# kocurvik/mdrp

Measured on AMD Instinct MI355X. Metric: image-pairs/sec (2000 corrs, 10k RANSAC iters), higher is better.
Workload: dtype f64

## Files before the change

### mdrp_amd/csrc/mdrp_capi.hip

```cpp
#include "../../include/mdrp.h"
#include "mdrp_kernels.h"
#include "mdrp_classic.h"
#ifdef MDRP_SPLIT_TU
#define MDRP_INST extern
#include "mdrp_instances.h"
namespace mdrp {
MDRP_INSTANCES_FINAL_64
MDRP_INSTANCES_FINAL_256
MDRP_INSTANCES_CLASSIC
}
#endif

#include <algorithm>
#include <cmath>
#include <cstdio>
#include <cstdlib>
#include <cstddef>
#include <cstring>
#include <functional>
#include <map>
#include <mutex>
#include <string>
#include <vector>

// ... 424 lines not shown
            int rc_;
            if ((rc_ = get_events(h, &v0, &v1, 5))) return rc_;
            HIPCHK(hipEventRecord(v0, st_));
            struct Stop { hipEvent_t e; hipStream_t s; ~Stop() { (void)hipEventRecord(e, s); } } stop_{v1, st_};
            PairState *st_p = h->st.as<PairState>() + p0;
            double *pts_p = h->pts.as<double>() + (size_t)p0 * n_max * PT_STRIDE;
            Model *models_p = h->models.as<Model>() + so;
            int32_t *inl_p = h->slot_inl.as<int32_t>() + so;
            if (classic) {
                const dim3 sgrid((r.chunk_len + 63) / 64, pc);
                if (kind == MDRP_SHARED_6PT)
                    hipLaunchKernelGGL(kc_solve<CLASSIC_SHARED>, sgrid, dim3(64), 0, st_, r, st_p, smp, pts_p, models_p, inl_p, tg, mc);
                else if (kind == MDRP_RELPOSE_5PT) {
                    const bool first_region = c == 0 && n_chunks > 1;
                    if (first_region && (size_t)sgrid.x > red5_first_blocks) { g_err = "5-point first chunk longer than its Reduce5 region"; return MDRP_ERR_INVALID; }
                    double *red5 = h->red5.as<double>() + ((first_region ? (size_t)batch * red5_blocks : 0) + (size_t)p0 * sgrid.x) * RED5_STRIDE * 64;
                    hipLaunchKernelGGL(kc_solve5_null, sgrid, dim3(64), SOLVE5N_LDS_BYTES, st_, r, st_p, smp, pts_p, red5);
                    hipLaunchKernelGGL(kc_solve5_reduce, sgrid, dim3(64), SOLVE5_LDS_BYTES, st_, r, st_p, red5);
                    hipLaunchKernelGGL(kc_solve5_roots, sgrid, dim3(64), SOLVE5B_LDS_BYTES, st_, r, st_p, smp, pts_p, red5, models_p, inl_p, tg, mc);
                }
                else
                    hipLaunchKernelGGL(kc_solve<CLASSIC_FUND>, sgrid, dim3(64), SOLVE7_LDS_BYTES, st_, r, st_p, smp, pts_p, models_p, inl_p, tg, mc);
                return MDRP_OK;
            }
            double *dep_p = h->dep.as<double>() + (size_t)p0 * n_max * 2;
#define MDRP_SOLVE_LAUNCH(S)                                                                                                   \
    hipLaunchKernelGGL(k_solve<S>, dim3((r.chunk_len + solve_threads(S) - 1) / solve_threads(S), pc), dim3(solve_threads(S)), 0, st_, r, st_p, smp, pts_p, dep_p, models_p, inl_p, tg, mc, 0, r.chunk_len)
            switch (r.solver) {
            case SOLVER_P3P: MDRP_SOLVE_LAUNCH(SOLVER_P3P); break;
            case SOLVER_SHIFT: MDRP_SOLVE_LAUNCH(SOLVER_SHIFT); break;
            case SOLVER_SHARED: MDRP_SOLVE_LAUNCH(SOLVER_SHARED); break;
            default: MDRP_SOLVE_LAUNCH(SOLVER_VARYING); break;
            }
#undef MDRP_SOLVE_LAUNCH
            return MDRP_OK;
        };
        auto sweep_chunk = [&](int c, int p0, int pc) -> int {
            RunParams r = rp;
            r.chunk_len = (int)lens[c]; r.chunk_off = offs[c]; r.batch = pc;
            const int len = r.chunk_len;
            const bool odd = c & 1;
            const size_t so = (size_t)p0 * rp.slot_stride;
            PairState *st_p = h->st.as<PairState>() + p0;
            const double *pts_p = h->pts.as<double>() + (size_t)p0 * n_max * PT_STRIDE;
            const Model *models_p = h->models.as<Model>() + so;
            uint32_t *tags_sc = (odd ? h->tags2_s : h->tags_s).as<uint32_t>() + so;
            int32_t *mcount_c = (odd ? h->model_count2 : h->model_count).as<int32_t>() + 2 * (size_t)p0;
            uint32_t *tags_c = (odd ? h->tags2 : h->tags).as<uint32_t>() + so;
            uint32_t *tags_v = h->tags_v.as<uint32_t>() + so;
            int32_t *surv1 = h->surv_count.as<int32_t>() + p0, *surv2 = h->surv2_count.as<int32_t>() + p0;
            hipEvent_t e0, e1;
            int rc_;
            if ((rc_ = get_events(h, &e0, &e1, 0))) return rc_;
            unsigned long long *cstats = reinterpret_cast<unsigned long long *>(cnt + 6);
            {
                hipEvent_t c0, c1;
                if ((rc_ = get_events(h, &c0, &c1, 1))) return rc_;
                const bool two_phase = !(it0 == 0 && c == 0);
                unsigned long long *cand_stat = h->cand_stat.as<unsigned long long>() + 2 * (size_t)p0;
                uint32_t *tags_u = tags_sc;
                int32_t *und_part = reinterpret_cast<int32_t *>((odd ? h->tags_s : h->tags2_s).as<uint32_t>() + so), *und_cnt = h->und_count.as<int32_t>() + 2 * (size_t)p0;
                const uint4 *rfrag_p = h->rfrag.as<uint4>() + (size_t)p0 * groups_max * 64;
                hipLaunchKernelGGL(k_count_plan, dim3(1), dim3(PLAN_THREADS), 0, s, pc, st_p, mcount_c, 2, CNT_WG_MODELS, h->cplan.as<int32_t>(),
                                   surv1, (const int32_t *)nullptr, two_phase ? und_cnt : (int32_t *)nullptr);
                const dim3 cgrid((unsigned)pc * (unsigned)((len * mps + CNT_WG_MODELS - 1) / CNT_WG_MODELS));
                HIPCHK(hipEventRecord(c0, s));
                MDRP_SWEEP_DISPATCH(k_count, kind, cgrid, dim3(CNT_THREADS), 0, s, r, st_p, rfrag_p, models_p,
                                    tags_c, mcount_c, h->cplan.as<int32_t>(), tags_v, surv1, cstats, (int32_t *)nullptr, (const int32_t *)nullptr,
                                    1, tags_u, und_part, und_cnt, (const int32_t *)nullptr, cand_stat);
                if (two_phase) {
                    hipLaunchKernelGGL(k_count_plan, dim3(1), dim3(PLAN_THREADS), 0, s, pc, st_p, und_cnt, 2, CNT_WG_MODELS, h->cplan.as<int32_t>(),
                                       (int32_t *)nullptr, (const int32_t *)nullptr, (int32_t *)nullptr);
                    MDRP_SWEEP_DISPATCH(k_count, kind, cgrid, dim3(CNT_THREADS), 0, s, r, st_p, rfrag_p, models_p,
                                        tags_u, und_cnt, h->cplan.as<int32_t>(), tags_v, surv1, cstats, (int32_t *)nullptr, (const int32_t *)nullptr,
                                        2, (uint32_t *)nullptr, (int32_t *)nullptr, (int32_t *)nullptr, und_part, cand_stat);
                    h->count_launches++;
                }
                HIPCHK(hipEventRecord(c1, s));
                h->count_launches++;
            }
            const uint32_t *surv_tags = tags_v;
            const int32_t *surv_cnt = surv1;
            if (use_bound && batch_call > 16 && !(it0 == 0 && c == 0)) {
                hipLaunchKernelGGL(k_count_plan, dim3(1), dim3(PLAN_THREADS), 0, s, pc, st_p, surv1, 1, BND_THREADS, h->cplan.as<int32_t>(), surv2, (const int32_t *)nullptr);
                const dim3 bgrid((unsigned)pc * (unsigned)((len * mps + BND_THREADS - 1) / BND_THREADS));
                unsigned long long *bstats = reinterpret_cast<unsigned long long *>(cnt + 12);
                hipEvent_t b0, b1;
                if ((rc_ = get_events(h, &b0, &b1, 4))) return rc_;
                HIPCHK(hipEventRecord(b0, s));
                MDRP_SWEEP_DISPATCH(k_bound, kind, bgrid, dim3(BND_THREADS), 0, s, r, st_p, pts_p, models_p, tags_v, surv1, h->cplan.as<int32_t>(), tags_c, surv2, bstats);
                HIPCHK(hipEventRecord(b1, s));
                surv_tags = tags_c; surv_cnt = surv2;
            }
            int32_t *plan = h->plan.as<int32_t>(), *totals = plan + 2 * (size_t)batch + 2;
            if (batch_call <= SCORE_WAVE_MAX_PAIRS) {
                hipLaunchKernelGGL(k_count_plan, dim3(1), dim3(PLAN_THREADS), 0, s, pc, st_p, surv_cnt, 1, SCW_THREADS / 64, plan, (int32_t *)nullptr, (const int32_t *)nullptr, (int32_t *)nullptr);
                hipLaunchKernelGGL(k_sort_tags, dim3(pc), dim3(256), 0, s, r, st_p, mcount_c, surv_cnt, surv_tags, tags_sc);
                HIPCHK(hipEventRecord(e0, s));
                const long long ub = (long long)pc * ((len * mps + SCW_THREADS / 64 - 1) / (SCW_THREADS / 64));
                const dim3 grid((unsigned)std::min<long long>(ub, (long long)h->num_cu * 32));
                MDRP_SWEEP_DISPATCH(k_score_w, kind, grid, dim3(SCW_THREADS), 0, s, r, st_p, pts_p, models_p, tags_sc, mcount_c,
                                    h->slot_score.as<double>() + so, h->slot_inl.as<int32_t>() + so, plan);
            } else {
                hipLaunchKernelGGL(k_sort_tags, dim3(pc), dim3(256), 0, s, r, st_p, mcount_c, surv_cnt, surv_tags, tags_sc);
                hipLaunchKernelGGL(k_plan, dim3(1), dim3(PLAN_THREADS), 0, s, pc, mcount_c, plan, totals);
                HIPCHK(hipEventRecord(e0, s));
                const dim3 grid((unsigned)pc * (unsigned)((len * mps + SCORE_THREADS - 1) / SCORE_THREADS));
                MDRP_SWEEP_DISPATCH(k_score, kind, grid, dim3(SCORE_THREADS), tile_bytes, s, r, st_p, pts_p, models_p, tags_sc, mcount_c,
                                    h->slot_score.as<double>() + so, h->slot_inl.as<int32_t>() + so, plan, totals);
            }
            HIPCHK(hipEventRecord(e1, s));
            h->sweep_launches++;
            Trigger *trig_p = h->triggers.as<Trigger>() + (size_t)p0 * trig_cap;
            unsigned long long *scan_stats = reinterpret_cast<unsigned long long *>(cnt + 10);
#define MDRP_SCAN(M, I) hipLaunchKernelGGL((k_scan<M, I>), dim3(pc), dim3(64), 0, s, r, st_p, h->slot_score.as<double>() + so, h->slot_inl.as<int32_t>() + so, trig_p, trig_cap, mcount_c, scan_stats)
            if (mps == 16) MDRP_SCAN(16, 1);
            else if (mps == 12) MDRP_SCAN(12, 1);
            else if (len >= 1024) MDRP_SCAN(4, 4);
            else MDRP_SCAN(4, 1);
#undef MDRP_SCAN
            return MDRP_OK;
        };
        bool solved1 = false;
        int swept0 = 0;
        if (host && it0 == 0) {
            const bool sliced = piped && n_chunks >= 2 && batch >= 2 * HOST_SLICE_PAIRS;
            const int sl = sliced ? HOST_SLICE_PAIRS : batch;
            for (int p0 = 0; p0 < batch; p0 += sl) {
                const int pc = std::min(sl, batch - p0);
                const size_t o2 = (size_t)2 * p0 * n_max, o1 = (size_t)p0 * n_max, n2 = sizeof(double) * 2 * (size_t)pc * n_max, n1 = sizeof(double) * (size_t)pc * n_max;
                hipStream_t cs = sliced ? h->copy_stream : s;
                HIPCHK(hipMemcpyAsync(const_cast<double *>(x1) + o2, host->x1 + o2, n2, hipMemcpyHostToDevice, cs));
                HIPCHK(hipMemcpyAsync(const_cast<double *>(x2) + o2, host->x2 + o2, n2, hipMemcpyHostToDevice, cs));
                if (host->d1 && host->d2) {
                    HIPCHK(hipMemcpyAsync(const_cast<double *>(d1) + o1, host->d1 + o1, n1, hipMemcpyHostToDevice, cs));
                    HIPCHK(hipMemcpyAsync(const_cast<double *>(d2) + o1, host->d2 + o1, n1, hipMemcpyHostToDevice, cs));
                }
                if (!sliced) { launch_prep(p0, pc, s); break; }
                HIPCHK(hipEventRecord(h->ev_copied, cs)); HIPCHK(hipStreamWaitEvent(aux, h->ev_copied, 0));
                if (p0 == 0) HIPCHK(hipStreamWaitEvent(aux, h->ev_tables, 0));
                launch_prep(p0, pc, aux);
                HIPCHK(hipEventRecord(h->ev_prepped, aux));
                if ((rc = issue_solve(1, aux, p0, pc))) return rc;
                const bool last = p0 + sl >= batch, last_but_one = !last && p0 + 2 * sl >= batch;
                if (last_but_one || last) HIPCHK(hipStreamWaitEvent(s, h->ev_prepped, 0));
                if (last_but_one) { swept0 = p0 + pc; if ((rc = issue_solve(0, s, 0, swept0)) || (rc = sweep_chunk(0, 0, swept0))) return rc; }
                if (last) { if ((rc = issue_solve(0, s, swept0, batch - swept0)) || (rc = sweep_chunk(0, swept0, batch - swept0))) return rc; swept0 = batch; }
            }
            if (sliced) { HIPCHK(hipEventRecord(h->ev_solved[1], aux)); solved1 = true; }
        }
        if (swept0 < batch && (rc = issue_solve(0, s, 0, batch))) return rc;
        if (piped) HIPCHK(hipEventRecord(h->ev_solved[0], s));
        for (int c = 0; c < n_chunks; ++c) {
            rp.chunk_len = (int)lens[c]; rp.chunk_off = offs[c];
            if (c == 0 && swept0 >= batch) {
                if (piped) HIPCHK(hipEventRecord(h->ev_scanned[0], s));
                continue;
            }
            if (piped && c + 1 < n_chunks && !(c == 0 && solved1)) {
                HIPCHK(hipStreamWaitEvent(aux, c == 0 ? h->ev_solved[0] : h->ev_scanned[c - 1], 0));
                if ((rc = issue_solve(c + 1, aux, 0, batch))) return rc;
                HIPCHK(hipEventRecord(h->ev_solved[c + 1], aux));
            }
            if (piped && c > 0) HIPCHK(hipStreamWaitEvent(s, h->ev_solved[c], 0));
            if (!piped && c > 0 && (rc = issue_solve(c, s, 0, batch))) return rc;
            if ((rc = sweep_chunk(c, 0, batch))) return rc;
            if (c + 1 < n_chunks) {
                if (piped) HIPCHK(hipEventRecord(h->ev_scanned[c], s));
                continue;
            }
            int32_t *lo_plan = h->work_pair.as<int32_t>();
            hipLaunchKernelGGL(k_lo_plan, dim3(1), dim3(PLAN_THREADS), 0, s, batch, h->st.as<PairState>(), (const int32_t *)nullptr, lo_plan);
            if (fuse_tail) {
// ... 683 lines not shown
```

### mdrp_amd/csrc/mdrp_kernels.h

```cpp
#pragma once
#include <hip/hip_runtime.h>
#include <float.h>
#include "mdrp_logtab.h"
#include "mdrp_math.h"

#ifdef MDRP_SECONDARY_TU
#define MDRP_GLOBAL static __global__
#else
#define MDRP_GLOBAL __global__
#endif

namespace mdrp {

constexpr int PT_STRIDE = 6;
#define MDRP_TILE_PTS 512
#define MDRP_SCORE_MINWAVES 4
constexpr int TILE_PTS = MDRP_TILE_PTS;
constexpr size_t SCORE_TILE_BYTES = (size_t)TILE_PTS * (PT_STRIDE * sizeof(double) + 4 * sizeof(float));
#define MDRP_P1F_UNROLL 8
#define MDRP_P1_UNROLL 4
constexpr int PRUNE_EVERY = 4;
#define MDRP_DENSE_KEY 40
#define MDRP_SOLVE_MINWAVES 2
#define MDRP_SCORE_THREADS 256
// ... 904 lines not shown
                if (g + 2 < A_TILE_GROUPS) {
#pragma unroll
                    for (int t = 0; t < CNT_TILES; t += 2) { test2(t); mfma2(f0, t); }
                } else {
#pragma unroll
                    for (int t = 0; t < CNT_TILES; t += 2) test2(t);
                }
            }
        }
        if (tile + 1 < t_hi) commit(buf ^ 1);
        __syncthreads();
    }
    if (idle) return;
    uint32_t *s_out = reinterpret_cast<uint32_t *>(&s_frag[wave][0][0]);
    const int swept = (t_hi - t_lo) * A_TILE_GROUPS * 16, real = min(max(n - t_lo * A_TILE_GROUPS * 16, 0), swept);
    const int pad = swept - real;
    const bool split_a = phase == 1 && t_hi < n_tiles;
    const int rest = split_a ? n - t_hi * A_TILE_GROUPS * 16 : 0;
#pragma unroll
    for (int t = 0; t < CNT_TILES; ++t) {
        float o = cand[t];
        o += __shfl_xor(o, 16, 64);
        o += __shfl_xor(o, 32, 64);
        if (ksl == 0) s_out[16 * t + col] = (uint32_t)((int)o - pad);
    }
    __builtin_amdgcn_fence(__ATOMIC_RELEASE, "wavefront");
    __builtin_amdgcn_wave_barrier();
    const long long rec_cnt = (long long)ps.best_min_cnt;
    const double rec_score = ps.best_min_score < DBL_MAX ? ps.best_min_score * (1.0 + 1e-12) : DBL_MAX;
#pragma unroll
    for (int r = 0; r < CNT_ROUNDS; ++r) {
        const int i = m0 + 64 * r + lane;
        const bool live = i < cnt;
        const int cnd_here = live ? (int)s_out[64 * r + lane] + part_r[r] : 0;
        const int cnd = cnd_here + rest;
        if (cand_stat && phase == 1 && !split_a && rec_cnt == 0 && !(ps.best_min_score < DBL_MAX)) {
            const int tot = wave_sum_i(cnd_here), lv = __popcll(__ballot(live));
            if (lane == 0 && lv) { atomicAdd(&cand_stat[2 * pair], (unsigned long long)tot); atomicAdd(&cand_stat[2 * pair + 1], (unsigned long long)lv * (unsigned long long)n); }
        }
        if (cand_out && live) cand_out[i] = cnd;
        const bool surv = live && ((long long)cnd > rec_cnt || thr * (double)(n - cnd) < rec_score);
        const unsigned long long ball = __ballot(surv);
        if (ball) {
            int base = 0;
            const int first = __ffsll((long long)ball) - 1;
            if (lane == first) base = atomicAdd(split_a ? &und_count[2 * pair] : &surv_count[pair], __popcll(ball));
            base = __shfl(base, first, 64);
            if (surv) {
                const size_t at = slot_base + base + __popcll(ball & ((1ull << lane) - 1ull));
                if (split_a) { tags_und[at] = slot_r[r]; und_part[at] = cnd_here; }
                else {
                    const uint32_t key = (uint32_t)min(PROBE_PTS, (int)(((long long)cnd * PROBE_PTS + n - 1) / n));
                    tags_surv[at] = slot_r[r] | (key << 24);
                }
            }
        }
    }
    if (stats && lane == 0 && wave == 0 && blk == 0) {
        if (phase != 2) atomicAdd(&stats[0], (unsigned long long)cnt * (unsigned long long)n);
        atomicAdd(&stats[1], (unsigned long long)(((cnt + 15) / 16) * 16) * (unsigned long long)swept);
    }
}

constexpr int BND_THREADS = 256;
#define MDRP_BND_TILE 256
constexpr int BND_TILE = MDRP_BND_TILE;

template <bool POSE, bool RAWF>
__device__ __forceinline__ void model_matrix(const Model &m, double E[9]) {
    if (RAWF) {
#pragma unroll
        for (int q = 0; q < 9; ++q) E[q] = reinterpret_cast<const double *>(&m)[q];
    } else {
        double R[9], Em[9];
        quat_to_R(m.q, R);
        essential_from_Rt(R, m.t, Em);
        if (POSE) {
#pragma unroll
            for (int q = 0; q < 9; ++q) E[q] = Em[q];
        } else fundamental_from_E(Em, m.f1, m.f2, E);
    }
}

template <bool POSE, bool RAWF = false>
__global__ __launch_bounds__(BND_THREADS, 4) void k_bound(RunParams rp, const PairState *__restrict__ st, const double *__restrict__ pts,
                                                          const Model *__restrict__ models, const uint32_t *__restrict__ tags_in,
                                                          const int32_t *__restrict__ cnt_in, const int32_t *__restrict__ plan,
                                                          uint32_t *__restrict__ tags_out,
                                                          int32_t *__restrict__ cnt_out, unsigned long long *__restrict__ stats,
                                                          double *__restrict__ dbg_lb = nullptr ,
                                                          int32_t *__restrict__ dbg_cnt_ub = nullptr) {
    __shared__ float4 s_rec[BND_TILE];
    struct Open { uint32_t tag; int32_t sane; float Ef[9], eC, eD, thr_dn, c0, c1; double lb; };
    __shared__ Open s_open[BND_THREADS];
    __shared__ int s_wave_open[BND_THREADS / 64];
    const int total = plan[rp.batch];
    const int w = blockIdx.x;
    if (w >= total) return;
    const int pair = plan_find(plan, rp.batch, w);
    const int blk = w - plan[pair];
    const PairState &ps = st[pair];
    const int n = ps.n, cnt = cnt_in[pair];
    const int tid = threadIdx.x, lane = tid & 63, wave = tid >> 6;
    const int i = blk * BND_THREADS + tid;
    bool open = i < cnt;
    const size_t slot_base = (size_t)pair * rp.slot_stride;
    const double thr = ps.sq_thr;
    uint32_t tag = 0;
    float Ef[9], eC = 0.f, eD = 1.f, thr_dn = 0.f;
    bool sane = false;
#pragma unroll
    for (int q = 0; q < 9; ++q) Ef[q] = 0.f;
    if (open) {
        tag = tags_in[slot_base + i];
        const Model m = models[slot_base + (tag & 0xFFFFFFu)];
        double E[9];
        model_matrix<POSE, RAWF>(m, E);
        sane = bound_setup32(E, ps.box, thr, Ef, eC, eD, thr_dn);
    }
    double total_lb = 0.0;
    f32x2 cnt2 = {0.f, 0.f};
    const float thr_cnt = (float)(thr * (1.0 + 1e-5)) * (1.0f + 1e-6f);
    const float BIG = 1.2089258e24f;
    const f32x2 nbig = {-BIG, -BIG}, kcnt = {thr_cnt * BIG, thr_cnt * BIG};
    const long long rec_cnt = (long long)ps.best_min_cnt;
    const double rec_score = ps.best_min_score < DBL_MAX ? ps.best_min_score * (1.0 + 1e-12) : DBL_MAX;
    float4 *s_pair = s_rec;
    const double *gp = pts + (size_t)pair * rp.n_max * PT_STRIDE;
    for (int t0 = 0; t0 < n; t0 += BND_TILE) {
        const int npts = min(BND_TILE, n - t0);
        __syncthreads();
        for (int j = tid; j < npts; j += BND_THREADS) {
            const double2 *src = reinterpret_cast<const double2 *>(gp + (size_t)(t0 + j) * PT_STRIDE);
            const double2 p0 = src[0], p1 = src[1];
            store_rec32(s_pair, j, p0.x, p0.y, p1.x, p1.y);
        }
        __syncthreads();
        if (__ballot(open)) {
            f32x2 Ev[9];
#pragma unroll
            for (int q = 0; q < 9; ++q) Ev[q] = (f32x2){Ef[q], Ef[q]};
            const f32x2 eDv = {eD, eD};
            const int npairs = npts >> 1;
            for (int j0 = 0; j0 < npairs; j0 += 32) {
                const int je = min(32, npairs - j0);
                f32x2 part = {0.f, 0.f};
#pragma unroll 2
                for (int j = 0; j < je; ++j) {
                    const float4 ab = s_pair[2 * (j0 + j)], cd = s_pair[2 * (j0 + j) + 1];
                    const f32x2 a = {ab.x, ab.y}, b = {ab.z, ab.w}, c = {cd.x, cd.y}, d = {cd.z, cd.w};
                    const f32x2 e0 = __builtin_elementwise_fma(Ev[0], a, __builtin_elementwise_fma(Ev[1], b, Ev[2]));
                    const f32x2 e1 = __builtin_elementwise_fma(Ev[3], a, __builtin_elementwise_fma(Ev[4], b, Ev[5]));
                    const f32x2 e2 = __builtin_elementwise_fma(Ev[6], a, __builtin_elementwise_fma(Ev[7], b, Ev[8]));
                    const f32x2 g0 = __builtin_elementwise_fma(Ev[0], c, __builtin_elementwise_fma(Ev[3], d, Ev[6]));
                    const f32x2 g1 = __builtin_elementwise_fma(Ev[1], c, __builtin_elementwise_fma(Ev[4], d, Ev[7]));
                    const f32x2 C = __builtin_elementwise_fma(c, e0, __builtin_elementwise_fma(d, e1, e2));
                    const f32x2 den = __builtin_elementwise_fma(e0, e0, __builtin_elementwise_fma(e1, e1, __builtin_elementwise_fma(g0, g0, __builtin_elementwise_fma(g1, g1, eDv))));
                    const f32x2 t = {fmaxf(fabsf(C.x) - eC, 0.0f), fmaxf(fabsf(C.y) - eC, 0.0f)};
                    const f32x2 rc = {__builtin_amdgcn_rcpf(den.x), __builtin_amdgcn_rcpf(den.y)};
                    const f32x2 q = (t * t) * rc;
                    const f32x2 term = {__builtin_fminf(q.x, thr_dn), __builtin_fminf(q.y, thr_dn)};
                    part += term;
                    f32x2 o;
                    asm("v_pk_fma_f32 %0, %1, %2, %3 clamp" : "=v"(o) : "v"(q), "v"(nbig), "v"(kcnt));
                    cnt2 += o;
                }
                total_lb += (double)part.x + (double)part.y;
            }
            if (npts & 1) {
                const float *fl = reinterpret_cast<const float *>(s_pair) + (npts >> 1) * 8;
                const float q = bound_r2_32(Ef, eC, eD, fl[0], fl[2], fl[4], fl[6]);
                total_lb += (double)__builtin_fminf(q, thr_dn);
                cnt2.x += (q < thr_cnt) ? 1.0f : 0.0f;
            }
        }
        const int seen = t0 + npts;
        if (open && sane) {
            const long long cnt_ub = (long long)(cnt2.x + cnt2.y) + 1 + (long long)(n - seen);
            if (cnt_ub <= rec_cnt && total_lb * (1.0 - BOUND_SLACK) >= rec_score) open = false;
        }
        if (seen >= n) break;
        const unsigned long long ob = __ballot(open);
        if (lane == 0) s_wave_open[wave] = __popcll(ob);
        __syncthreads();
        int tot = 0, before = 0, waves_used = 0;
#pragma unroll
        for (int v = 0; v < BND_THREADS / 64; ++v) { const int c = s_wave_open[v]; if (v < wave) before += c; tot += c; waves_used += c > 0; }
        if (tot == 0) break;
        if ((tot + 63) / 64 < waves_used) {
            if (open) {
                Open &o = s_open[before + __popcll(ob & ((1ull << lane) - 1ull))];
                o.tag = tag; o.sane = sane; o.eC = eC; o.eD = eD; o.thr_dn = thr_dn; o.c0 = cnt2.x; o.c1 = cnt2.y; o.lb = total_lb;
#pragma unroll
                for (int q = 0; q < 9; ++q) o.Ef[q] = Ef[q];
            }
            __syncthreads();
            open = tid < tot;
            if (open) {
                const Open &o = s_open[tid];
                tag = o.tag; sane = o.sane != 0; eC = o.eC; eD = o.eD; thr_dn = o.thr_dn; cnt2.x = o.c0; cnt2.y = o.c1; total_lb = o.lb;
#pragma unroll
                for (int q = 0; q < 9; ++q) Ef[q] = o.Ef[q];
            }
        }
    }
    const bool surv = open;
    if (dbg_lb && surv) {
        dbg_lb[tag & 0xFFFFFFu] = sane ? total_lb * (1.0 - BOUND_SLACK) : 0.0;
        dbg_cnt_ub[tag & 0xFFFFFFu] = sane ? (int32_t)min((long long)n, (long long)(cnt2.x + cnt2.y) + 1) : n;
    }
    const unsigned long long ball = __ballot(surv);
    if (ball) {
        int base = 0;
        const int first = __ffsll((long long)ball) - 1;
        if (lane == first) base = atomicAdd(&cnt_out[pair], __popcll(ball));
        base = __shfl(base, first, 64);
        if (surv) tags_out[slot_base + base + __popcll(ball & ((1ull << lane) - 1ull))] = tag;
    }
    if (stats && tid == 0 && blk == 0) atomicAdd(stats, (unsigned long long)cnt * (unsigned long long)n);
}

MDRP_GLOBAL __launch_bounds__(256) void k_sort_tags(RunParams rp, const PairState *__restrict__ st, int32_t *__restrict__ model_count,
                                                   const int32_t *__restrict__ surv_count,
                                                   const uint32_t *__restrict__ tags, uint32_t *__restrict__ tags_sorted) {
    const int pair = blockIdx.x, tid = threadIdx.x;
    const PairState &ps = st[pair];
    if (!ps.active) return;
    __shared__ int s_hist[PROBE_PTS + 1], s_pos[PROBE_PTS + 1];
    __shared__ int s_dense;
    if (tid <= PROBE_PTS) s_hist[tid] = 0;
    if (tid == 0) s_dense = 0;
    __syncthreads();
    const int cnt = surv_count[pair];
    const size_t slot_base = (size_t)pair * rp.slot_stride;
    const uint32_t *src = tags + slot_base;
    uint32_t *dst = tags_sorted + slot_base;
    const int dense_min = ps.n >= 8 ? MDRP_DENSE_KEY : PROBE_PTS + 1;
    for (int i = tid; i < cnt; i += 256) atomicAdd(&s_hist[min(src[i] >> 24, (uint32_t)PROBE_PTS)], 1);
    __syncthreads();
    if (tid < 64) {
        const int v = tid < dense_min ? s_hist[tid] : 0;
        int incl = v;
#pragma unroll
        for (int o = 1; o < 64; o <<= 1) {
            const int u = __shfl_up(incl, o, 64);
            if (tid >= o) incl += u;
        }
        s_pos[tid] = incl - v;
        if (tid == 63) s_pos[64] = incl;
    }
    __syncthreads();
    const int cap = rp.slot_stride;
    for (int i = tid; i < cnt; i += 256) {
        const uint32_t t = src[i];
        const int key = (int)min(t >> 24, (uint32_t)PROBE_PTS);
        if (key >= dense_min) dst[cap - 1 - atomicAdd(&s_dense, 1)] = t & 0xFFFFFFu;
        else dst[atomicAdd(&s_pos[key], 1)] = t & 0xFFFFFFu;
    }
    __syncthreads();
    if (tid == 0) { model_count[2 * pair] = cnt - s_dense; model_count[2 * pair + 1] = s_dense; }
}

MDRP_GLOBAL __launch_bounds__(PLAN_THREADS) void k_plan(int batch, const int32_t *__restrict__ model_count, int32_t *__restrict__ plan,
                                                       int32_t *__restrict__ totals ) {
    __shared__ int s_w[PLAN_THREADS / 64 + 1];
    int run_d = 0, run_s = 0;
    int32_t *pd = plan, *psp = plan + batch + 1;
    for (int p0 = 0; p0 < batch; p0 += PLAN_THREADS) {
        const int p = p0 + threadIdx.x;
        int bd = 0, bs = 0;
        if (p < batch) {
            bs = (model_count[2 * p] + SCORE_THREADS - 1) / SCORE_THREADS;
            bd = (model_count[2 * p + 1] + SCORE_THREADS - 1) / SCORE_THREADS;
        }
        int tot_d, tot_s;
        const int ed = plan_block_scan(bd, tot_d, s_w), es = plan_block_scan(bs, tot_s, s_w);
        if (p < batch) { pd[p] = run_d + run_s + ed + es; psp[p] = bs; }
        run_d += tot_d;
        run_s += tot_s;
    }
    if (threadIdx.x == 0) { pd[batch] = run_d + run_s; psp[batch] = 0; totals[0] = run_d; totals[1] = run_d + run_s; totals[2] = 0; }
}

template <bool POSE, bool RAWF = false>
__global__ __launch_bounds__(SCORE_THREADS, MDRP_SCORE_MINWAVES) void k_score(RunParams rp, const PairState *__restrict__ st, const double *__restrict__ pts,
                                                         const Model *__restrict__ models, const uint32_t *__restrict__ tags,
                                                         const int32_t *__restrict__ model_count, double *__restrict__ slot_score,
                                                         int32_t *__restrict__ slot_inl, const int32_t *__restrict__ plan,
                                                         int32_t *__restrict__ totals) {
    extern __shared__ double tile[];
    float4 *tile32 = reinterpret_cast<float4 *>(tile + TILE_PTS * PT_STRIDE);
    const int total = totals[1];
    const int tid = threadIdx.x;
// ... 1047 lines not shown
```

### mdrp_amd/csrc/mdrp_math.h

```cpp
#pragma once
#include <math.h>
#include <stdint.h>

#if defined(__HIPCC__)
#define MDRP_HD __host__ __device__ __forceinline__
#else
#define MDRP_HD inline
#endif

namespace mdrp {

struct Model {
    double q[4];
    double t[3];
    double scale, shift1, shift2;
    double f1, f2;
};

MDRP_HD void model_identity(Model &m) {
    m.q[0] = 1.0; m.q[1] = 0.0; m.q[2] = 0.0; m.q[3] = 0.0;
    m.t[0] = 0.0; m.t[1] = 0.0; m.t[2] = 0.0;
    m.scale = 1.0; m.shift1 = 0.0; m.shift2 = 0.0; m.f1 = 1.0; m.f2 = 1.0;
}

// ... 776 lines not shown

MDRP_HD void count_setup(const double E[9], const double box[4], double thr, uint16_t eh[8], uint16_t el[8], uint16_t e8[3], float &tb) {
    const double ax = box[0], ay = box[1], cx = box[2], cy = box[3];
    const double e0 = fabs(E[0]) * ax + fabs(E[1]) * ay + fabs(E[2]), e1 = fabs(E[3]) * ax + fabs(E[4]) * ay + fabs(E[5]);
    const double g0 = fabs(E[0]) * cx + fabs(E[3]) * cy + fabs(E[6]), g1 = fabs(E[1]) * cx + fabs(E[4]) * cy + fabs(E[7]);
    const double dmax = (1.0 + 1e-9) * (e0 * e0 + e1 * e1 + g0 * g0 + g1 * g1);
    const double e2 = fabs(E[6]) * ax + fabs(E[7]) * ay + fabs(E[8]);
    const double M = e0 * cx + e1 * cy + e2;
    const double T = sqrt(thr * (1.0 + 1e-12) * dmax);
    tb = (M < 1e30) ? (float)((T + COUNT_KAPPA * M) * (1.0 + 1e-6)) + 1e-30f : __builtin_inff();
    for (int j = 0; j < 8; ++j) bf16_split(E[j], eh[j], el[j]);
    bf16_split3(E[8], e8[0], e8[1], e8[2]);
}

MDRP_HD void bf16_split_f32(float x, uint16_t &h, uint16_t &l) {
    h = bf16_bits(x);
    l = bf16_bits(x - bf16_value(h));
}
MDRP_HD void count_setup_scaled(const double E[9], const double box[4], double thr, uint16_t eh[8], uint16_t el[8], uint16_t e8[3], float &tb2) {
    const double ax = box[0], ay = box[1], cx = box[2], cy = box[3];
    const double e0 = fabs(E[0]) * ax + fabs(E[1]) * ay + fabs(E[2]), e1 = fabs(E[3]) * ax + fabs(E[4]) * ay + fabs(E[5]);
    const double g0 = fabs(E[0]) * cx + fabs(E[3]) * cy + fabs(E[6]), g1 = fabs(E[1]) * cx + fabs(E[4]) * cy + fabs(E[7]);
    const double dmax = (1.0 + 1e-9) * (e0 * e0 + e1 * e1 + g0 * g0 + g1 * g1);
    const double e2 = fabs(E[6]) * ax + fabs(E[7]) * ay + fabs(E[8]);
    const double M = e0 * cx + e1 * cy + e2;
    const float td = (float)(thr * (1.0 + 1e-12) * dmax), km = (float)(COUNT_KAPPA * M);
    const float tb = (sqrtf(td) + km) * (1.0f + 1e-6f) + 1e-30f;
    for (int j = 0; j < 8; ++j) { eh[j] = 0; el[j] = 0; }
    e8[0] = e8[1] = e8[2] = 0;
    tb2 = 1.0f;
    if (!(M < 1e30) || !(tb < 1e30f) || !(tb > 0.0f) || !(td > 1e-30f) || !(km > 1e-30f)) return;
    int ex;
    (void)frexpf(tb, &ex);
    const int k = 21 - ex;
    const double S = ldexp(1.0, k);
    for (int j = 0; j < 8; ++j) bf16_split_f32((float)(E[j] * S), eh[j], el[j]);
    const float c8 = (float)(E[8] * S);
    bf16_split_f32(c8, e8[0], e8[1]);
    e8[2] = bf16_bits((c8 - bf16_value(e8[0])) - bf16_value(e8[1]));
    const float tbs = ldexpf(tb, k);
    tb2 = (tbs * tbs) * (1.0f + 2e-7f);
}

constexpr double BOUND_SLACK = 2e-5;

MDRP_HD bool bound_setup32(const double E[9], const double box[4], double thr, float Ef[9], float &eC, float &eD, float &thr_dn) {
    const double ax = box[0], ay = box[1], cx = box[2], cy = box[3];
    const double e0 = fabs(E[0]) * ax + fabs(E[1]) * ay + fabs(E[2]), e1 = fabs(E[3]) * ax + fabs(E[4]) * ay + fabs(E[5]);
    const double g0 = fabs(E[0]) * cx + fabs(E[3]) * cy + fabs(E[6]), g1 = fabs(E[1]) * cx + fabs(E[4]) * cy + fabs(E[7]);
    const double dmax = e0 * e0 + e1 * e1 + g0 * g0 + g1 * g1;
    const double e2 = fabs(E[6]) * ax + fabs(E[7]) * ay + fabs(E[8]);
    const double M = e0 * cx + e1 * cy + e2;
    const bool sane = (M < 1e15) && (dmax < 1e30) && (dmax > 1e-30);
    eC = sane ? (float)(2e-6 * M * (1.0 + 1e-6)) + 1e-30f : 0.0f;
    eD = sane ? (float)(4e-6 * dmax * (1.0 + 1e-6)) + 1e-37f : 1.0f;
    float t = (float)thr;
    if ((double)t > thr && t > 0.0f) {
        uint32_t bits;
        __builtin_memcpy(&bits, &t, 4);
        --bits;
        __builtin_memcpy(&t, &bits, 4);
    }
    thr_dn = t;
    for (int i = 0; i < 9; ++i) Ef[i] = (float)E[i];
    return sane;
}

MDRP_HD float bound_r2_32(const float Ef[9], float eC, float eD, float a, float b, float c, float d) {
    const float e0 = fmaf(Ef[0], a, fmaf(Ef[1], b, Ef[2]));
    const float e1 = fmaf(Ef[3], a, fmaf(Ef[4], b, Ef[5]));
    const float e2 = fmaf(Ef[6], a, fmaf(Ef[7], b, Ef[8]));
    const float g0 = fmaf(Ef[0], c, fmaf(Ef[3], d, Ef[6]));
    const float g1 = fmaf(Ef[1], c, fmaf(Ef[4], d, Ef[7]));
    const float C = fmaf(c, e0, fmaf(d, e1, e2));
    const float den = fmaf(e0, e0, fmaf(e1, e1, fmaf(g0, g0, fmaf(g1, g1, eD))));
    const float t = fmaxf(fabsf(C) - eC, 0.0f);
#if defined(__HIP_DEVICE_COMPILE__)
    return (t * t) * __builtin_amdgcn_rcpf(den);
#else
    return (t * t) / den;
#endif
}

struct LmState {
    double R[9], t[3], s, u, v, f1, f2;
    double E[9], F[9];
    double if1, if2;
};

MDRP_HD void lm_state_from_model(const Model &m, bool focal, LmState &st) {
    quat_to_R(m.q, st.R);
    st.t[0] = m.t[0]; st.t[1] = m.t[1]; st.t[2] = m.t[2];
    st.s = m.scale; st.u = m.shift1; st.v = m.shift2;
    st.f1 = focal ? m.f1 : 1.0; st.f2 = focal ? m.f2 : 1.0;
    st.if1 = 1.0 / st.f1; st.if2 = 1.0 / st.f2;
    essential_from_Rt(st.R, st.t, st.E);
    fundamental_from_E(st.E, st.f1, st.f2, st.F);
}

constexpr int LM_NPAR = 11;

template <bool WITH_J, bool FOCAL>
MDRP_HD void lm_sampson_term(const LmState &st, double x1x, double x1y, double x2x, double x2y, double &r0, double *J0) {
    const double *R = st.R, *F = FOCAL ? st.F : st.E, *E = st.E;
    const double f1 = FOCAL ? st.f1 : 1.0, f2 = FOCAL ? st.f2 : 1.0;
    const double Fh1_0 = F[0] * x1x + F[1] * x1y + F[2], Fh1_1 = F[3] * x1x + F[4] * x1y + F[5], Fh1_2 = F[6] * x1x + F[7] * x1y + F[8];
    const double Ft2_0 = F[0] * x2x + F[3] * x2y + F[6], Ft2_1 = F[1] * x2x + F[4] * x2y + F[7];
    const double C = x2x * Fh1_0 + x2y * Fh1_1 + Fh1_2;
    const double den = Fh1_0 * Fh1_0 + Fh1_1 * Fh1_1 + Ft2_0 * Ft2_0 + Ft2_1 * Ft2_1;
    const double isd = lm_rsqrt(den);
    r0 = C * isd;
    if (!WITH_J) return;
    const double h1[3] = {x1x, x1y, 1.0}, h2[3] = {x2x, x2y, 1.0};
    const double Fh1[3] = {Fh1_0, Fh1_1, Fh1_2}, Ft2[3] = {Ft2_0, Ft2_1, 0.0};
    const double k = C * isd * isd * isd;
    double GE[9];
    double G[9];
#pragma unroll
    for (int i = 0; i < 3; ++i)
#pragma unroll
        for (int j = 0; j < 3; ++j) {
            double g = h2[i] * h1[j] * isd;
            if (i < 2) g -= k * Fh1[i] * h1[j];
            if (j < 2) g -= k * Ft2[j] * h2[i];
            G[3 * i + j] = g;
            GE[3 * i + j] = g * (i == 2 ? f2 : 1.0) * (j == 2 ? f1 : 1.0);
        }
#pragma unroll
    for (int a = 0; a < 3; ++a) {
        const int b = (a + 1) % 3, c = (a + 2) % 3;
        double acc = 0;
#pragma unroll
        for (int i = 0; i < 3; ++i) acc += GE[3 * i + b] * E[3 * i + c] - GE[3 * i + c] * E[3 * i + b];
        J0[a] = acc;
        double acc2 = 0;
#pragma unroll
        for (int j = 0; j < 3; ++j) acc2 += -GE[3 * b + j] * R[3 * c + j] + GE[3 * c + j] * R[3 * b + j];
        J0[3 + a] = acc2;
    }
    J0[6] = 0; J0[7] = 0; J0[8] = 0;
    J0[9] = G[2] * E[2] + G[5] * E[5] + G[8] * E[8] * f2;
    J0[10] = G[6] * E[6] + G[7] * E[7] + G[8] * E[8] * f1;
}

template <bool WITH_J, bool FOCAL>
MDRP_HD void lm_forward_term(const LmState &st, double sqrt_sr, double x1x, double x1y, double x2x, double x2y, double d1,
                             double &r1, double &r2, double &zf, double *J1, double *J2) {
    const double *R = st.R, *t = st.t;
    const double f2 = FOCAL ? st.f2 : 1.0;
    const double if1 = FOCAL ? st.if1 : 1.0;
    const double b1x = x1x * if1, b1y = x1y * if1;
    const double dd1 = d1 + st.u;
    const double X1[3] = {dd1 * b1x, dd1 * b1y, dd1};
    const double Z0 = R[0] * X1[0] + R[1] * X1[1] + R[2] * X1[2] + t[0];
    const double Z1 = R[3] * X1[0] + R[4] * X1[1] + R[5] * X1[2] + t[1];
    const double Z2 = R[6] * X1[0] + R[7] * X1[1] + R[8] * X1[2] + t[2];
    const double iz = lm_rcp(Z2);
    r1 = sqrt_sr * (f2 * Z0 * iz - x2x);
    r2 = sqrt_sr * (f2 * Z1 * iz - x2y);
    zf = Z2;
    if (!WITH_J) return;
    const double px0 = sqrt_sr * f2 * iz, pz0 = -sqrt_sr * f2 * Z0 * iz * iz, pz1 = -sqrt_sr * f2 * Z1 * iz * iz;
    const double cr[3][3] = {{0.0, -X1[2], X1[1]}, {X1[2], 0.0, -X1[0]}, {-X1[1], X1[0], 0.0}};
#pragma unroll
    for (int a = 0; a < 3; ++a) {
        const double v0 = R[0] * cr[a][0] + R[1] * cr[a][1] + R[2] * cr[a][2];
// ... 183 lines not shown
```

Measured before the change: 125,100.

## Add MFMA bf16-split bound kernel and route pairs between fp32 and matrix paths

Adds a new bound-pruning kernel that computes the epipolar numerator and denominator terms for 64 models per wave as bf16 matrix products, using v_mfma_f32_16x16x32_bf16 with three-way bf16 splitting to keep fp32-like accuracy. Each pair is routed either to this MFMA kernel or to the existing scalar fp32 k_bound, depending on how large the best inlier count is relative to n. Both kernels are launched and each exits early for pairs it does not own. The aim is to move the heavy per-model, per-point bound arithmetic onto matrix cores. The cost is an extra kernel launch, hand-written asm, and conservative error padding that could make pruning weaker.

Measured after the change: 128,400 (median of 6 runs). 2.7% higher.

```diff
diff --git a/mdrp_amd/csrc/mdrp_capi.hip b/mdrp_amd/csrc/mdrp_capi.hip
--- a/mdrp_amd/csrc/mdrp_capi.hip
+++ b/mdrp_amd/csrc/mdrp_capi.hip
@@ -530,13 +530,16 @@
             const uint32_t *surv_tags = tags_v;
             const int32_t *surv_cnt = surv1;
             if (use_bound && batch_call > 16 && !(it0 == 0 && c == 0)) {
-                hipLaunchKernelGGL(k_count_plan, dim3(1), dim3(PLAN_THREADS), 0, s, pc, st_p, surv1, 1, BND_THREADS, h->cplan.as<int32_t>(), surv2, (const int32_t *)nullptr);
-                const dim3 bgrid((unsigned)pc * (unsigned)((len * mps + BND_THREADS - 1) / BND_THREADS));
+                hipLaunchKernelGGL(k_count_plan, dim3(1), dim3(PLAN_THREADS), 0, s, pc, st_p, surv1, 1, MB_WG_MODELS, h->cplan.as<int32_t>(), surv2, (const int32_t *)nullptr);
+                const dim3 bgrid((unsigned)pc * (unsigned)((len * mps + MB_WG_MODELS - 1) / MB_WG_MODELS));
                 unsigned long long *bstats = reinterpret_cast<unsigned long long *>(cnt + 12);
                 hipEvent_t b0, b1;
                 if ((rc_ = get_events(h, &b0, &b1, 4))) return rc_;
                 HIPCHK(hipEventRecord(b0, s));
-                MDRP_SWEEP_DISPATCH(k_bound, kind, bgrid, dim3(BND_THREADS), 0, s, r, st_p, pts_p, models_p, tags_v, surv1, h->cplan.as<int32_t>(), tags_c, surv2, bstats);
+                MDRP_SWEEP_DISPATCH(k_mfma_bound, kind, bgrid, dim3(MB_THREADS), 0, s, r, st_p, pts_p, models_p, tags_v, surv1, h->cplan.as<int32_t>(), tags_c, surv2, bstats);
+                static_assert(MB_WG_MODELS == BND_THREADS, "the two bound kernels share one plan");
+                MDRP_SWEEP_DISPATCH(k_bound, kind, bgrid, dim3(BND_THREADS), 0, s, r, st_p, pts_p, models_p, tags_v, surv1, h->cplan.as<int32_t>(), tags_c, surv2, bstats,
+                                    (double *)nullptr, (int32_t *)nullptr, 1);
                 HIPCHK(hipEventRecord(b1, s));
                 surv_tags = tags_c; surv_cnt = surv2;
             }
diff --git a/mdrp_amd/csrc/mdrp_kernels.h b/mdrp_amd/csrc/mdrp_kernels.h
--- a/mdrp_amd/csrc/mdrp_kernels.h
+++ b/mdrp_amd/csrc/mdrp_kernels.h
@@ -1010,6 +1010,8 @@
     }
 }
 
+__device__ __forceinline__ bool bound_in_fp32(const PairState &ps) { return (long long)ps.best_min_cnt * 10 > (long long)ps.n * 7; }
+
 template <bool POSE, bool RAWF = false>
 __global__ __launch_bounds__(BND_THREADS, 4) void k_bound(RunParams rp, const PairState *__restrict__ st, const double *__restrict__ pts,
                                                           const Model *__restrict__ models, const uint32_t *__restrict__ tags_in,
@@ -1017,7 +1019,8 @@
                                                           uint32_t *__restrict__ tags_out,
                                                           int32_t *__restrict__ cnt_out, unsigned long long *__restrict__ stats,
                                                           double *__restrict__ dbg_lb = nullptr ,
-                                                          int32_t *__restrict__ dbg_cnt_ub = nullptr) {
+                                                          int32_t *__restrict__ dbg_cnt_ub = nullptr,
+                                                          int routed = 0 ) {
     __shared__ float4 s_rec[BND_TILE];
     struct Open { uint32_t tag; int32_t sane; float Ef[9], eC, eD, thr_dn, c0, c1; double lb; };
     __shared__ Open s_open[BND_THREADS];
@@ -1028,6 +1031,7 @@
     const int pair = plan_find(plan, rp.batch, w);
     const int blk = w - plan[pair];
     const PairState &ps = st[pair];
+    if (routed && !bound_in_fp32(ps)) return;
     const int n = ps.n, cnt = cnt_in[pair];
     const int tid = threadIdx.x, lane = tid & 63, wave = tid >> 6;
     const int i = blk * BND_THREADS + tid;
@@ -1137,6 +1141,212 @@
         dbg_lb[tag & 0xFFFFFFu] = sane ? total_lb * (1.0 - BOUND_SLACK) : 0.0;
         dbg_cnt_ub[tag & 0xFFFFFFu] = sane ? (int32_t)min((long long)n, (long long)(cnt2.x + cnt2.y) + 1) : n;
     }
+    const unsigned long long ball = __ballot(surv);
+    if (ball) {
+        int base = 0;
+        const int first = __ffsll((long long)ball) - 1;
+        if (lane == first) base = atomicAdd(&cnt_out[pair], __popcll(ball));
+        base = __shfl(base, first, 64);
+        if (surv) tags_out[slot_base + base + __popcll(ball & ((1ull << lane) - 1ull))] = tag;
+    }
+    if (stats && tid == 0 && blk == 0) atomicAdd(stats, (unsigned long long)cnt * (unsigned long long)n);
+}
+
+constexpr int MB_TILES = 4;
+constexpr int MB_THREADS = 256;
+constexpr int MB_WAVE_MODELS = 16 * MB_TILES;
+constexpr int MB_WG_MODELS = MB_WAVE_MODELS * (MB_THREADS / 64);
+constexpr int MB_GROUPS = MB_THREADS / 16;
+constexpr int MB_TILE_RECS = 16 * MB_GROUPS;
+
+template <bool POSE, bool RAWF = false>
+__global__ __launch_bounds__(MB_THREADS, 3) void k_mfma_bound(RunParams rp, const PairState *__restrict__ st, const double *__restrict__ pts,
+                                                              const Model *__restrict__ models, const uint32_t *__restrict__ tags_in,
+                                                              const int32_t *__restrict__ cnt_in, const int32_t *__restrict__ plan,
+                                                              uint32_t *__restrict__ tags_out, int32_t *__restrict__ cnt_out,
+                                                              unsigned long long *__restrict__ stats) {
+    __shared__ uint4 s_lds[MB_GROUPS * 3 * 64];
+    __shared__ int s_open[MB_THREADS / 64];
+    static_assert(MB_WG_MODELS * 4 <= MB_GROUPS * 3 * 64, "B staging fits the A tile");
+    const int total = plan[rp.batch];
+    const int w = blockIdx.x;
+    if (w >= total) return;
+    const int pair = plan_find(plan, rp.batch, w);
+    const int blk = w - plan[pair];
+    const PairState &ps = st[pair];
+    if (bound_in_fp32(ps)) return;
+    const int n = ps.n, cnt = cnt_in[pair];
+    const int tid = threadIdx.x, lane = tid & 63, wave = tid >> 6;
+    const int col = lane & 15, ksl = lane >> 4;
+    const int i = blk * MB_WG_MODELS + wave * MB_WAVE_MODELS + lane;
+    const bool live = i < cnt;
+    const size_t slot_base = (size_t)pair * rp.slot_stride;
+    const double thr = ps.sq_thr;
+    uint32_t tag = 0;
+    bool sane = false;
+    float eC = 0.0f;
+    bf16x8_t bC[MB_TILES], bS[MB_TILES], bD[MB_TILES];
+    {
+        uint16_t bc[32], bs[32], bd[32];
+        if (live) {
+            tag = tags_in[slot_base + i];
+            double E[9];
+            model_matrix<POSE, RAWF>(models[slot_base + (tag & 0xFFFFFFu)], E);
+            sane = mbound_setup(E, ps.box, thr, bc, bs, bd, eC);
+        } else {
+#pragma unroll
+            for (int k = 0; k < 32; ++k) { bc[k] = 0; bs[k] = 0; bd[k] = 0; }
+            bd[30] = 0x3F80;
+        }
+        uint4 *dst = s_lds + (size_t)(wave * MB_WAVE_MODELS + lane) * 4;
+#pragma unroll
+        for (int part = 0; part < 3; ++part) {
+            const uint16_t *b = part == 0 ? bc : part == 1 ? bs : bd;
+#pragma unroll
+            for (int k = 0; k < 4; ++k) dst[k] = pack_bf16x8(b + 8 * k);
+            __syncthreads();
+#pragma unroll
+            for (int t = 0; t < MB_TILES; ++t) {
+                const bf16x8_t v = __builtin_bit_cast(bf16x8_t, s_lds[(size_t)(wave * MB_WAVE_MODELS + 16 * t + col) * 4 + ksl]);
+                if (part == 0) bC[t] = v; else if (part == 1) bS[t] = v; else bD[t] = v;
+            }
+            __syncthreads();
+        }
+    }
+    float ec[MB_TILES], sum[MB_TILES], cntf[MB_TILES];
+    double lb[MB_TILES];
+    bool open[MB_TILES];
+    const long long rec_cnt = (long long)ps.best_min_cnt;
+    const double rec_score = ps.best_min_score < DBL_MAX ? ps.best_min_score * (1.0 + 1e-12) : DBL_MAX;
+#pragma unroll
+    for (int t = 0; t < MB_TILES; ++t) {
+        ec[t] = __shfl(eC, 16 * t + col, 64);
+        open[t] = __shfl((int)(live && sane), 16 * t + col, 64) != 0;
+        lb[t] = 0.0;
+        cntf[t] = 0.0f;
+    }
+    bool wave_open = __ballot(live && sane) != 0;
+    const float BIG = 1.2089258e24f;
+    f32x4_t accC[MB_TILES], accD[MB_TILES], accS[MB_TILES];
+    auto small1 = [&](const uint4 &sraw, int t) {
+        asm volatile("v_mfma_f32_16x16x32_bf16 %0, %1, %2, 0" : "=&v"(accS[t]) : "v"(__builtin_bit_cast(bf16x8_t, sraw)), "v"(bS[t]));
+    };
+    auto big2 = [&](const uint4 &craw, const uint4 &draw, int t) {
+        asm volatile("v_mfma_f32_16x16x32_bf16 %0, %3, %5, %2\n\t"
+                     "v_mfma_f32_16x16x32_bf16 %1, %4, %6, 0"
+                     : "=&v"(accC[t]), "=&v"(accD[t]) : "v"(accS[t]), "v"(__builtin_bit_cast(bf16x8_t, craw)),
+                       "v"(__builtin_bit_cast(bf16x8_t, draw)), "v"(bC[t]), "v"(bD[t]));
+    };
+    auto test = [&](int t) {
+        float q0, q1, q2, q3, r0, r1, r2, r3;
+        asm volatile("v_sub_f32_e64 %2, |%10|, %18 clamp\n\t"
+                     "v_sub_f32_e64 %3, |%11|, %18 clamp\n\t"
+                     "v_sub_f32_e64 %4, |%12|, %18 clamp\n\t"
+                     "v_sub_f32_e64 %5, |%13|, %18 clamp\n\t"
+                     "v_rcp_f32 %6, %14\n\t"
+                     "v_rcp_f32 %7, %15\n\t"
+                     "v_rcp_f32 %8, %16\n\t"
+                     "v_rcp_f32 %9, %17\n\t"
+                     "v_mul_f32 %2, %2, %2\n\t"
+                     "v_mul_f32 %3, %3, %3\n\t"
+                     "v_mul_f32 %4, %4, %4\n\t"
+                     "v_mul_f32 %5, %5, %5\n\t"
+                     "v_mul_f32_e64 %2, %2, %6 clamp\n\t"
+                     "v_mul_f32_e64 %3, %3, %7 clamp\n\t"
+                     "v_mul_f32_e64 %4, %4, %8 clamp\n\t"
+                     "v_mul_f32_e64 %5, %5, %9 clamp\n\t"
+                     "v_fma_f32 %6, %2, -%19, %19 clamp\n\t"
+                     "v_fma_f32 %7, %3, -%19, %19 clamp\n\t"
+                     "v_fma_f32 %8, %4, -%19, %19 clamp\n\t"
+                     "v_fma_f32 %9, %5, -%19, %19 clamp\n\t"
+                     "v_add_f32 %2, %2, %3\n\t"
+                     "v_add_f32 %4, %4, %5\n\t"
+                     "v_add_f32 %6, %6, %7\n\t"
+                     "v_add_f32 %8, %8, %9\n\t"
+                     "v_add_f32 %0, %0, %2\n\t"
+                     "v_add_f32 %1, %1, %6\n\t"
+                     "v_add_f32 %0, %0, %4\n\t"
+                     "v_add_f32 %1, %1, %8"
+                     : "+v"(sum[t]), "+v"(cntf[t]), "=&v"(q0), "=&v"(q1), "=&v"(q2), "=&v"(q3), "=&v"(r0), "=&v"(r1), "=&v"(r2), "=&v"(r3)
+                     : "v"(accC[t][0]), "v"(accC[t][1]), "v"(accC[t][2]), "v"(accC[t][3]), "v"(accD[t][0]), "v"(accD[t][1]),
+                       "v"(accD[t][2]), "v"(accD[t][3]), "v"(ec[t]), "v"(BIG));
+    };
+    const double *gp = pts + (size_t)pair * rp.n_max * PT_STRIDE;
+    for (int t0 = 0; t0 < n; t0 += MB_TILE_RECS) {
+        if (lane == 0) s_open[wave] = wave_open;
+        __syncthreads();
+        bool any = false;
+#pragma unroll
+        for (int v = 0; v < MB_THREADS / 64; ++v) any |= s_open[v] != 0;
+        if (!any) break;
+        {
+            uint16_t ac[32], as[32], ad[32];
+            const int rr = tid, r = t0 + rr;
+            double a = 0.0, b = 0.0, c = 0.0, d = 0.0;
+            if (r < n) {
+                const double2 *src = reinterpret_cast<const double2 *>(gp + (size_t)r * PT_STRIDE);
+                const double2 p0 = src[0], p1 = src[1];
+                a = p0.x; b = p0.y; c = p1.x; d = p1.y;
+            }
+            mbound_record(a, b, c, d, ac, as, ad);
+            uint4 *g = s_lds + (size_t)(rr >> 4) * 192 + (rr & 15);
+            const bool past_n = r >= n;
+#pragma unroll
+            for (int k = 0; k < 4; ++k) {
+                g[16 * k] = past_n ? make_uint4(0u, 0u, 0u, 0u) : pack_bf16x8(ac + 8 * k);
+                g[64 + 16 * k] = past_n ? make_uint4(0u, 0u, 0u, 0u) : pack_bf16x8(as + 8 * k);
+                g[128 + 16 * k] = pack_bf16x8(ad + 8 * k);
+            }
+        }
+        __syncthreads();
+        if (!wave_open) continue;
+#pragma unroll
+        for (int t = 0; t < MB_TILES; ++t) sum[t] = 0.0f;
+        {
+            const uint4 *T = s_lds + lane;
+            uint4 fc = T[0], fd = T[128], fs = T[64];
+#pragma unroll
+            for (int t = 0; t < MB_TILES; ++t) small1(fs, t);
+            asm volatile("s_nop 7\n\ts_nop 7\n\ts_nop 7" ::: "memory");
+#pragma unroll
+            for (int t = 0; t < MB_TILES; ++t) big2(fc, fd, t);
+            fs = T[192 + 64];
+#pragma unroll
+            for (int t = 0; t < MB_TILES; ++t) small1(fs, t);
+#pragma unroll
+            for (int g = 1; g <= MB_GROUPS; ++g) {
+                if (g < MB_GROUPS) { fc = T[(size_t)g * 192]; fd = T[(size_t)g * 192 + 128]; }
+                if (g + 1 < MB_GROUPS) fs = T[(size_t)(g + 1) * 192 + 64];
+#pragma unroll
+                for (int t = 0; t < MB_TILES; ++t) {
+                    test(t);
+                    if (g < MB_GROUPS) big2(fc, fd, t);
+                    if (g + 1 < MB_GROUPS) small1(fs, t);
+                }
+            }
+        }
+        const int seen = min(n, t0 + MB_TILE_RECS), past = t0 + MB_TILE_RECS - seen;
+#pragma unroll
+        for (int t = 0; t < MB_TILES; ++t) {
+            double s = (double)sum[t];
+            s += __shfl_xor(s, 16, 64);
+            s += __shfl_xor(s, 32, 64);
+            lb[t] += s;
+            float c = cntf[t];
+            c += __shfl_xor(c, 16, 64);
+            c += __shfl_xor(c, 32, 64);
+            const long long cnt_ub = (long long)c - past + (long long)(n - seen);
+            if (open[t] && cnt_ub <= rec_cnt && thr * lb[t] * (1.0 - BOUND_SLACK) >= rec_score) open[t] = false;
+        }
+        bool o = false;
+#pragma unroll
+        for (int t = 0; t < MB_TILES; ++t) o |= open[t];
+        wave_open = __ballot(o) != 0;
+    }
+    bool surv = false;
+#pragma unroll
+    for (int t = 0; t < MB_TILES; ++t) if (ksl == t) surv = open[t];
+    surv = live && (surv || !sane);
     const unsigned long long ball = __ballot(surv);
     if (ball) {
         int base = 0;
diff --git a/mdrp_amd/csrc/mdrp_math.h b/mdrp_amd/csrc/mdrp_math.h
--- a/mdrp_amd/csrc/mdrp_math.h
+++ b/mdrp_amd/csrc/mdrp_math.h
@@ -882,6 +882,78 @@
 #endif
 }
 
+constexpr double MBOUND_KAPPA_C = 1e-5;
+constexpr double MBOUND_KAPPA_D = 1e-4;
+constexpr double MBOUND_DELTA = 1e-5;
+constexpr double MBOUND_FLOOR = 8.673617379884035e-19;
+
+MDRP_HD void bf16_split3_f32(float x, uint16_t &h, uint16_t &l, uint16_t &l2) {
+    bf16_split_f32(x, h, l);
+    l2 = bf16_bits((x - bf16_value(h)) - bf16_value(l));
+}
+
+MDRP_HD bool mbound_setup(const double E[9], const double box[4], double thr, uint16_t bc[32], uint16_t bs[32], uint16_t bd[32], float &eC) {
+    const double ax = box[0], ay = box[1], cx = box[2], cy = box[3];
+    const double e0 = fabs(E[0]) * ax + fabs(E[1]) * ay + fabs(E[2]), e1 = fabs(E[3]) * ax + fabs(E[4]) * ay + fabs(E[5]);
+    const double g0 = fabs(E[0]) * cx + fabs(E[3]) * cy + fabs(E[6]), g1 = fabs(E[1]) * cx + fabs(E[4]) * cy + fabs(E[7]);
+    const double dmax = e0 * e0 + e1 * e1 + g0 * g0 + g1 * g1;
+    const double e2 = fabs(E[6]) * ax + fabs(E[7]) * ay + fabs(E[8]);
+    const double M = e0 * cx + e1 * cy + e2;
+    for (int k = 0; k < 32; ++k) { bc[k] = 0; bs[k] = 0; bd[k] = 0; }
+    bd[30] = 0x3F80;
+    eC = 0.0f;
+    if (!(M < 1e15) || !(M > 1e-30) || !(dmax < 1e30) || !(dmax > 1e-30) || !(thr > 0.0) || !(thr < 1e30)) return false;
+    int ex;
+    (void)frexp(M, &ex);
+    const double S = ldexp(1.0, -1 - ex);
+    const double sd = S * S * (thr * (1.0 + MBOUND_DELTA));
+    const double ds = dmax * sd * (1.0 + 1e-12);
+    if (!(ds > 9.094947017729282e-13) || !(ds < 1.099511627776e12)) return false;
+    double D[11];
+    D[0] = E[0] * E[0] + E[3] * E[3]; D[1] = 2.0 * (E[0] * E[1] + E[3] * E[4]); D[2] = E[1] * E[1] + E[4] * E[4];
+    D[3] = 2.0 * (E[0] * E[2] + E[3] * E[5]); D[4] = 2.0 * (E[1] * E[2] + E[4] * E[5]);
+    D[5] = E[0] * E[0] + E[1] * E[1]; D[6] = 2.0 * (E[0] * E[3] + E[1] * E[4]); D[7] = E[3] * E[3] + E[4] * E[4];
+    D[8] = 2.0 * (E[0] * E[6] + E[1] * E[7]); D[9] = 2.0 * (E[3] * E[6] + E[4] * E[7]);
+    D[10] = E[2] * E[2] + E[5] * E[5] + E[6] * E[6] + E[7] * E[7];
+    const double eD = MBOUND_KAPPA_D * ds * (1.0 + 2.0 * MBOUND_KAPPA_D) + MBOUND_FLOOR;
+    float cs[9], dsc[11];
+    for (int j = 0; j < 9; ++j) cs[j] = (float)(E[j] * S);
+    for (int j = 0; j < 11; ++j) dsc[j] = (float)(D[j] * sd + (j == 10 ? eD : 0.0));
+    for (int j = 0; j < 9; ++j) if (!(fabsf(cs[j]) <= 1.099511627776e12f)) return false;
+    for (int j = 0; j < 11; ++j) if (!(fabsf(dsc[j]) <= 1.099511627776e12f)) return false;
+    uint16_t h, l, l2;
+    for (int j = 0; j < 8; ++j) {
+        bf16_split3_f32(cs[j], h, l, l2);
+        bc[j] = h; bc[8 + j] = h; bc[16 + j] = l;
+        bs[j] = l; bs[8 + j] = h; bs[16 + j] = l2;
+    }
+    bf16_split3_f32(cs[8], bc[24], bc[25], bc[26]);
+    for (int j = 0; j < 10; ++j) { bf16_split_f32(dsc[j], h, l); bd[j] = h; bd[10 + j] = h; bd[20 + j] = l; }
+    bf16_split_f32(dsc[10], bd[30], bd[31]);
+    eC = (float)(MBOUND_KAPPA_C * M * S * (1.0 + 1e-6) + MBOUND_FLOOR);
+    return true;
+}
+
+MDRP_HD void mbound_record(double a, double b, double c, double d, uint16_t ac[32], uint16_t as[32], uint16_t ad[32]) {
+    for (int k = 0; k < 32; ++k) { ac[k] = 0; as[k] = 0; ad[k] = 0; }
+    ad[30] = ad[31] = 0x3F80;
+    const float af = (float)a, bf = (float)b, cf = (float)c, df = (float)d;
+    const float m[8] = {af * cf, bf * cf, cf, af * df, bf * df, df, af, bf};
+    const float p[10] = {af * af, af * bf, bf * bf, af, bf, cf * cf, cf * df, df * df, cf, df};
+    float mag = 0.0f;
+    for (int j = 0; j < 8; ++j) mag = fmaxf(mag, fabsf(m[j]));
+    for (int j = 0; j < 10; ++j) mag = fmaxf(mag, fabsf(p[j]));
+    if (!(mag < 1e15f) || !(af + bf + cf + df == af + bf + cf + df)) return;
+    uint16_t h, l, l2;
+    for (int j = 0; j < 8; ++j) {
+        bf16_split3_f32(m[j], h, l, l2);
+        ac[j] = h; ac[8 + j] = l; ac[16 + j] = h;
+        as[j] = l; as[8 + j] = l2; as[16 + j] = h;
+    }
+    ac[24] = ac[25] = ac[26] = 0x3F80;
+    for (int j = 0; j < 10; ++j) { bf16_split_f32(p[j], h, l); ad[j] = h; ad[10 + j] = l; ad[20 + j] = h; }
+}
+
 struct LmState {
     double R[9], t[3], s, u, v, f1, f2;
     double E[9], F[9];
```
